# Zanue/EndoDAV

Measured on AMD Instinct MI355X. Metric: depth frames/sec (518x518, T=8 clip), higher is better.
Workload: dtype f32

## Files before the change

endodav_amd/csrc/temporal.hip:

```cpp
#include <cstdlib>

#include "ops.hpp"

namespace edv {
namespace {

using f32x4 = __attribute__((ext_vector_type(4))) float;

template <int TMAX>
__global__ __launch_bounds__(256) void attn_temporal_kernel(const float *__restrict__ qkv, float *__restrict__ out, int B, int T, int P, int C,
                                                             int heads, float scale) {
    const long long total = (long long)B * T * P * heads;
    const long long gid = (long long)blockIdx.x * 256 + threadIdx.x;
    if (gid >= total) return;
    const int head = (int)(gid % heads);
    long long r = gid / heads;
    const int p = (int)(r % P);
    r /= P;
    const int tq = (int)(r % T);
    const int b = (int)(r / T);
    const int d = C / heads, C3 = 3 * C;
    const long long tstride = (long long)P * C3;
    const float *qp = qkv + ((long long)(b * T + tq) * P + p) * C3 + head * d;
    const float *kb = qkv + ((long long)(b * T) * P + p) * C3 + C + head * d;
    const float *vb = kb + C;

    float s[TMAX];
#pragma unroll
    for (int ts = 0; ts < TMAX; ++ts) s[ts] = 0.f;
    for (int c = 0; c < d; c += 4) {
        const f32x4 q4 = *reinterpret_cast<const f32x4 *>(qp + c);
#pragma unroll
        for (int ts = 0; ts < TMAX; ++ts) {
            if (ts < T) {
                const f32x4 k4 = *reinterpret_cast<const f32x4 *>(kb + ts * tstride + c);
                s[ts] += (q4.x * k4.x + q4.y * k4.y) + (q4.z * k4.z + q4.w * k4.w);
            }
        }
    }
    float mx = -INFINITY;
#pragma unroll
    for (int ts = 0; ts < TMAX; ++ts)
        if (ts < T) {
            s[ts] *= scale;
            mx = fmaxf(mx, s[ts]);
        }
    float sum = 0.f;
#pragma unroll
    for (int ts = 0; ts < TMAX; ++ts)
        if (ts < T) {
            s[ts] = expf(s[ts] - mx);
            sum += s[ts];
        }
    const float inv = 1.0f / sum;
    float *op = out + ((long long)(b * T + tq) * P + p) * C + head * d;
    for (int c = 0; c < d; c += 4) {
        f32x4 acc = {0.f, 0.f, 0.f, 0.f};
#pragma unroll
        for (int ts = 0; ts < TMAX; ++ts)
            if (ts < T) acc += s[ts] * *reinterpret_cast<const f32x4 *>(vb + ts * tstride + c);
        *reinterpret_cast<f32x4 *>(op + c) = acc * inv;
    }
}

template <int TT>
__global__ __launch_bounds__(256) void attn_temporal_small_kernel(const float *__restrict__ qkv, float *__restrict__ out, int B, int T, int P, int C, int heads,
                                                                   float scale) {
    const long long total = (long long)B * P * heads;
    const long long gid = (long long)blockIdx.x * 256 + threadIdx.x;
    if (gid >= total) return;
    const int head = (int)(gid % heads);
    long long r = gid / heads;
    const int p = (int)(r % P);
    const int b = (int)(r / P);
    const int d = C / heads, C3 = 3 * C;
    const long long ts3 = (long long)P * C3, ts1 = (long long)P * C;
    const float *qb = qkv + ((long long)(b * T) * P + p) * C3 + head * d;
    const float *kb = qb + C, *vb = qb + 2 * C;
    float *ob = out + ((long long)(b * T) * P + p) * C + head * d;
    float S[TT][TT];
#pragma unroll
    for (int i = 0; i < TT; ++i)
#pragma unroll
        for (int j = 0; j < TT; ++j) S[i][j] = 0.f;
#pragma unroll 2
    for (int c = 0; c < d; c += 4) {
        f32x4 q4[TT], k4[TT];
#pragma unroll
        for (int t = 0; t < TT; ++t) {
            const int tc = t < T ? t : T - 1;
            q4[t] = *reinterpret_cast<const f32x4 *>(qb + tc * ts3 + c);
            k4[t] = *reinterpret_cast<const f32x4 *>(kb + tc * ts3 + c);
        }
#pragma unroll
        for (int i = 0; i < TT; ++i)
#pragma unroll
            for (int j = 0; j < TT; ++j) S[i][j] += (q4[i].x * k4[j].x + q4[i].y * k4[j].y) + (q4[i].z * k4[j].z + q4[i].w * k4[j].w);
    }
#pragma unroll
    for (int i = 0; i < TT; ++i) {
        float mx = -INFINITY;
#pragma unroll
        for (int j = 0; j < TT; ++j)
            if (j < T) {
                S[i][j] *= scale;
                mx = fmaxf(mx, S[i][j]);
            }
        float sum = 0.f;
#pragma unroll
        for (int j = 0; j < TT; ++j) {
            S[i][j] = j < T ? expf(S[i][j] - mx) : 0.f;
            sum += S[i][j];
        }
        const float inv = 1.0f / sum;
#pragma unroll
        for (int j = 0; j < TT; ++j) S[i][j] *= inv;
    }
#pragma unroll 2
    for (int c = 0; c < d; c += 4) {
        f32x4 v4[TT];
#pragma unroll
        for (int t = 0; t < TT; ++t) v4[t] = *reinterpret_cast<const f32x4 *>(vb + (t < T ? t : T - 1) * ts3 + c);
#pragma unroll
        for (int i = 0; i < TT; ++i) {
            if (i < T) {
                f32x4 acc = {0.f, 0.f, 0.f, 0.f};
#pragma unroll
                for (int j = 0; j < TT; ++j) acc += S[i][j] * v4[j];
                *reinterpret_cast<f32x4 *>(ob + i * ts1 + c) = acc;
            }
        }
    }
}

template <int TMAX>
__global__ __launch_bounds__(256) void attn_temporal_pixel_kernel(const float *__restrict__ qkv, float *__restrict__ out, int T, int P, int C, int heads,
                                                                   int HG, float scale) {
    extern __shared__ __attribute__((aligned(16))) float sm[];
    const int tid = threadIdx.x, nthr = blockDim.x;
    const int ngroups = heads / HG;
    const int hg = blockIdx.x % ngroups;
    const long long bp = blockIdx.x / ngroups;
    const int b = (int)(bp / P), p = (int)(bp - (long long)b * P);
    const int d = C / heads, C3 = 3 * C, W = HG * d, w4 = W >> 2;
    for (int idx = tid; idx < T * 3 * w4; idx += nthr) {
        const int t = idx / (3 * w4), r = idx - t * 3 * w4;
        const int part = r / w4, c4 = r - part * w4;
        *reinterpret_cast<f32x4 *>(&sm[(t * 3 + part) * W + 4 * c4]) =
            *reinterpret_cast<const f32x4 *>(qkv + ((long long)(b * T + t) * P + p) * C3 + part * C + hg * W + 4 * c4);
    }
    __syncthreads();
    const int hl = tid % HG, tq = tid / HG;
    if (tq >= T) return;
    const float *q = sm + (tq * 3 + 0) * W + hl * d;
    float s[TMAX];
#pragma unroll
    for (int ts = 0; ts < TMAX; ++ts) s[ts] = 0.f;
    for (int c = 0; c < d; c += 4) {
        const f32x4 q4 = *reinterpret_cast<const f32x4 *>(q + c);
#pragma unroll
        for (int ts = 0; ts < TMAX; ++ts)
            if (ts < T) {
                const f32x4 k4 = *reinterpret_cast<const f32x4 *>(sm + (ts * 3 + 1) * W + hl * d + c);
                s[ts] += (q4.x * k4.x + q4.y * k4.y) + (q4.z * k4.z + q4.w * k4.w);
            }
    }
    float mx = -INFINITY;
#pragma unroll
    for (int ts = 0; ts < TMAX; ++ts)
        if (ts < T) {
            s[ts] *= scale;
            mx = fmaxf(mx, s[ts]);
        }
    float sum = 0.f;
#pragma unroll
    for (int ts = 0; ts < TMAX; ++ts) {
        s[ts] = ts < T ? expf(s[ts] - mx) : 0.f;
        sum += s[ts];
    }
    const float inv = 1.0f / sum;
    float *op = out + ((long long)(b * T + tq) * P + p) * C + (hg * HG + hl) * d;
    for (int c = 0; c < d; c += 4) {
        f32x4 acc = {0.f, 0.f, 0.f, 0.f};
#pragma unroll
        for (int ts = 0; ts < TMAX; ++ts)
            if (ts < T) acc += s[ts] * *reinterpret_cast<const f32x4 *>(sm + (ts * 3 + 2) * W + hl * d + c);
        *reinterpret_cast<f32x4 *>(op + c) = acc * inv;
    }
}

__global__ __launch_bounds__(256) void geglu_kernel(const float *__restrict__ x, float *__restrict__ y, long long total4, int inner4) {
    for (long long i = (long long)blockIdx.x * 256 + threadIdx.x; i < total4; i += (long long)gridDim.x * 256) {
        const long long m = i / inner4;
        const int j = (int)(i - m * inner4);
        const float *row = x + m * (long long)inner4 * 8;
        const f32x4 a = *reinterpret_cast<const f32x4 *>(row + 4 * j);
        const f32x4 g = *reinterpret_cast<const f32x4 *>(row + 4 * (inner4 + j));
        f32x4 o = {a.x * gelu_erf(g.x), a.y * gelu_erf(g.y), a.z * gelu_erf(g.z), a.w * gelu_erf(g.w)};
        *reinterpret_cast<f32x4 *>(y + i * 4) = o;
    }
}


__global__ __launch_bounds__(256) void rope_qk_kernel(float *__restrict__ qkv, const float *__restrict__ table, long long n_pairs, int T, int P, int C,
                                                      float sign) {
    const long long i = (long long)blockIdx.x * 256 + threadIdx.x;
    if (i >= n_pairs) return;
    const int half = C >> 1;
    const long long m = i / half;
    const int j = (int)(i - m * half);
    const int t = (int)((m / P) % T);
    const float2 cs = *reinterpret_cast<const float2 *>(table + ((size_t)t * half + j) * 2);
    const float c = cs.x, sn = sign * cs.y;
    float2 *q = reinterpret_cast<float2 *>(qkv + m * 3 * C + 2 * j), *k = reinterpret_cast<float2 *>(qkv + m * 3 * C + C + 2 * j);
    const float2 a = *q, b = *k;
    *q = make_float2(a.x * c - a.y * sn, a.x * sn + a.y * c);
    *k = make_float2(b.x * c - b.y * sn, b.x * sn + b.y * c);
}

}

int attn_temporal(const float *qkv, float *out, int B, int T, int P, int C, int heads, hipStream_t st) {
    EDV_CHECK(qkv && out, "null operand");
    EDV_CHECK(B > 0 && T > 0 && P > 0 && C > 0 && heads > 0, "empty problem");
    EDV_CHECK(T <= 64, "T > 64 frames per clip is not built (temporal attention keeps a query's T scores in registers)");
    EDV_CHECK(C % heads == 0 && (C / heads) % 4 == 0, "head dim must be a multiple of 4");
    const long long total = (long long)B * T * P * heads;
    const long long blocks = (total + 255) / 256;
    EDV_CHECK(blocks < (1ll << 31), "grid");
    const float scale = 1.0f / sqrtf((float)(C / heads));
    dim3 grid((unsigned)blocks), block(256);
    static const bool per_query = [] {
        const char *e = getenv("EDV_TATTN_PER_QUERY");
        return e && atoi(e) != 0;
    }();
    const int d = C / heads;
    int HG = heads;
    while (HG > 1 && ((long long)T * HG > 256 || (size_t)T * 3 * HG * d * sizeof(float) > 64 * 1024 || heads % HG != 0)) --HG;
    const size_t lds_cap = (T > 32 && HG == 1) ? 160 * 1024 : 64 * 1024;
    const bool pixel_fits = (long long)T * HG <= 256 && (size_t)T * 3 * HG * d * sizeof(float) <= lds_cap && (long long)B * P * (heads / HG) < (1ll << 31);
    if (!per_query && pixel_fits && (T > 8 || d >= 24)) {
        const dim3 g3((unsigned)((long long)B * P * (heads / HG)));
        const dim3 b3((unsigned)(((T * HG + 63) / 64) * 64));
        const size_t lds = (size_t)T * 3 * HG * d * sizeof(float);
        if (T <= 8)
            EDV_LAUNCH(attn_temporal_pixel_kernel<8>, g3, b3, lds, st, qkv, out, T, P, C, heads, HG, scale);
        else if (T <= 16)
            EDV_LAUNCH(attn_temporal_pixel_kernel<16>, g3, b3, lds, st, qkv, out, T, P, C, heads, HG, scale);
        else if (T <= 32)
            EDV_LAUNCH(attn_temporal_pixel_kernel<32>, g3, b3, lds, st, qkv, out, T, P, C, heads, HG, scale);
        else {
            if (lds > 64 * 1024)
                EDV_HIP(hipFuncSetAttribute(reinterpret_cast<const void *>(attn_temporal_pixel_kernel<64>), hipFuncAttributeMaxDynamicSharedMemorySize, (int)lds_cap));
            EDV_LAUNCH(attn_temporal_pixel_kernel<64>, g3, b3, lds, st, qkv, out, T, P, C, heads, HG, scale);
        }
    } else if (T > 32) {
        EDV_CHECK(false, "temporal attention over more than 32 frames: one head's q|k|v of a pixel (T x 3 x C/8 floats) must fit the 160 KB of LDS");
    } else if (T <= 8 && !per_query) {
        const long long tot = (long long)B * P * heads;
        const dim3 g2((unsigned)((tot + 255) / 256));
        if (T <= 4)
            EDV_LAUNCH(attn_temporal_small_kernel<4>, g2, block, 0, st, qkv, out, B, T, P, C, heads, scale);
        else
            EDV_LAUNCH(attn_temporal_small_kernel<8>, g2, block, 0, st, qkv, out, B, T, P, C, heads, scale);
    } else if (T <= 8)
        EDV_LAUNCH(attn_temporal_kernel<8>, grid, block, 0, st, qkv, out, B, T, P, C, heads, scale);
    else if (T <= 16)
        EDV_LAUNCH(attn_temporal_kernel<16>, grid, block, 0, st, qkv, out, B, T, P, C, heads, scale);
    else
        EDV_LAUNCH(attn_temporal_kernel<32>, grid, block, 0, st, qkv, out, B, T, P, C, heads, scale);
    EDV_LAUNCH_OK();
    return 0;
}

int geglu(const float *x, float *y, long long M, int inner, hipStream_t st) {
    EDV_CHECK(x && y, "null operand");
    EDV_CHECK(M > 0 && inner > 0 && inner % 4 == 0, "shape");
    const long long total4 = M * (inner / 4);
    const int blocks = (int)((total4 + 255) / 256 < 8192 ? (total4 + 255) / 256 : 8192);
    EDV_LAUNCH(geglu_kernel, dim3(blocks), dim3(256), 0, st, x, y, total4, inner / 4);
    EDV_LAUNCH_OK();
    return 0;
}

int rope_qk(float *qkv, const float *table, int B, int T, int P, int C, bool transpose, hipStream_t st) {
    EDV_CHECK(qkv && table, "null operand");
    EDV_CHECK(B > 0 && T > 0 && P > 0 && C > 0 && C % 2 == 0, "bad shape");
    const long long n = (long long)B * T * P * (C / 2);
    EDV_LAUNCH(rope_qk_kernel, dim3((unsigned)((n + 255) / 256)), dim3(256), 0, st, qkv, table, n, T, P, C, transpose ? -1.f : 1.f);
    EDV_LAUNCH_OK();
    return 0;
}

}
```

Measured before the change: 1027.

## Add pixel-tiled temporal attention kernel staging multiple pixels per block in LDS

Adds a new temporal attention kernel that loads a tile of up to eight pixels times a group of heads for all T frames into shared memory. Loads are issued into registers before any LDS write, giving wider, more coalesced global reads. Each query's head dimension is split across several lanes, and the partial dot products are combined with xor shuffles. It is enabled by default through an env knob and replaces the previous one-pixel-per-block kernel, at the cost of more register pressure and extra index math.

New measurement: 1032, median of 6. Within noise of the previous version (+0.5%).

```diff
diff --git a/endodav_amd/csrc/temporal.hip b/endodav_amd/csrc/temporal.hip
--- a/endodav_amd/csrc/temporal.hip
+++ b/endodav_amd/csrc/temporal.hip
@@ -189,6 +189,93 @@
     }
 }
 
+__device__ __forceinline__ int div_small(int a, float inv) { return (int)(((float)a + 0.5f) * inv); }
+
+template <int TMAX, int NL>
+__global__ __launch_bounds__(256, TMAX == 32 ? 3 : 1) void attn_temporal_tile_kernel(const float *__restrict__ qkv, float *__restrict__ out, int T, int P, int C,
+                                                                                      int heads, int lpt, int lhg, int lsp, int tiles, int rs4, float inv_rw4,
+                                                                                      float inv_w4, float scale) {
+    extern __shared__ __attribute__((aligned(16))) f32x4 sm4[];
+    const int tid = threadIdx.x;
+    const int PT = 1 << lpt, HG = 1 << lhg, DS = 1 << lsp;
+    const int ngroups = heads >> lhg;
+    const int hg = blockIdx.x % ngroups;
+    const int bt = blockIdx.x / ngroups;
+    const int b = bt / tiles, p0 = (bt - b * tiles) << lpt;
+    const int d4 = (C / heads) >> 2, c4n = C >> 2, w4 = d4 << lhg, rw4 = 3 * w4;
+    const int n4 = (T << lpt) * rw4;
+    const f32x4 *src = reinterpret_cast<const f32x4 *>(qkv) + (long long)b * T * P * (3 * c4n) + hg * w4;
+    f32x4 v[NL];
+    int dst[NL];
+#pragma unroll
+    for (int i = 0; i < NL; ++i) {
+        const int slot = tid + i * 256;
+        const int idx = slot < n4 ? slot : n4 - 1;
+        const int row = div_small(idx, inv_rw4), r = idx - row * rw4;
+        const int part = div_small(r, inv_w4), c4 = r - part * w4;
+        const int t = row >> lpt, pp = p0 + (row & (PT - 1));
+        const int pc = pp < P ? pp : P - 1;
+        dst[i] = (slot < n4 && pp < P) ? row * rs4 + part * w4 + c4 : -1;
+        v[i] = src[((long long)t * P + pc) * (3 * c4n) + part * c4n + c4];
+    }
+#pragma unroll
+    for (int i = 0; i < NL; ++i)
+        if (dst[i] >= 0) sm4[dst[i]] = v[i];
+    __syncthreads();
+    const int nwork = T << (lpt + lhg + lsp), fs4 = rs4 << lpt;
+    for (int it = tid; it < nwork; it += 256) {
+        const int ds = it & (DS - 1), hl = (it >> lsp) & (HG - 1), pix = (it >> (lsp + lhg)) & (PT - 1), tq = it >> (lsp + lhg + lpt);
+        const int pp = p0 + pix;
+        if (pp >= P) continue;
+        const f32x4 *base = sm4 + pix * rs4 + hl * d4;
+        const f32x4 *q = base + tq * fs4;
+        float s[TMAX];
+#pragma unroll
+        for (int ts = 0; ts < TMAX; ++ts) s[ts] = 0.f;
+        for (int c = ds; c < d4; c += DS) {
+            const f32x4 q4 = q[c];
+#pragma unroll
+            for (int t0 = 0; t0 < TMAX; t0 += 8)
+                if (t0 < T) {
+#pragma unroll
+                    for (int ts = t0; ts < t0 + 8; ++ts) {
+                        const f32x4 k4 = base[(ts < T ? ts : T - 1) * fs4 + w4 + c];
+                        s[ts] += (q4.x * k4.x + q4.y * k4.y) + (q4.z * k4.z + q4.w * k4.w);
+                    }
+                }
+        }
+        for (int m = 1; m < DS; m <<= 1) {
+#pragma unroll
+            for (int ts = 0; ts < TMAX; ++ts) s[ts] += __shfl_xor(s[ts], m);
+        }
+        float mx = -INFINITY;
+#pragma unroll
+        for (int ts = 0; ts < TMAX; ++ts)
+            if (ts < T) {
+                s[ts] *= scale;
+                mx = fmaxf(mx, s[ts]);
+            }
+        float sum = 0.f;
+#pragma unroll
+        for (int ts = 0; ts < TMAX; ++ts) {
+            s[ts] = ts < T ? expf(s[ts] - mx) : 0.f;
+            sum += s[ts];
+        }
+        const float inv = 1.0f / sum;
+        f32x4 *op = reinterpret_cast<f32x4 *>(out) + ((long long)(b * T + tq) * P + pp) * c4n + ((hg << lhg) + hl) * d4;
+        for (int c = ds; c < d4; c += DS) {
+            f32x4 acc = {0.f, 0.f, 0.f, 0.f};
+#pragma unroll
+            for (int t0 = 0; t0 < TMAX; t0 += 8)
+                if (t0 < T) {
+#pragma unroll
+                    for (int ts = t0; ts < t0 + 8; ++ts) acc += s[ts] * base[(ts < T ? ts : T - 1) * fs4 + 2 * w4 + c];
+                }
+            op[c] = acc * inv;
+        }
+    }
+}
+
 __global__ __launch_bounds__(256) void geglu_kernel(const float *__restrict__ x, float *__restrict__ y, long long total4, int inner4) {
     for (long long i = (long long)blockIdx.x * 256 + threadIdx.x; i < total4; i += (long long)gridDim.x * 256) {
         const long long m = i / inner4;
@@ -218,6 +305,58 @@
     *k = make_float2(b.x * c - b.y * sn, b.x * sn + b.y * c);
 }
 
+constexpr size_t TILE_LDS = 48 * 1024;
+struct TilePlan {
+    int lpt, lhg, lsp, rs4, tiles, nl;
+    size_t bytes;
+    long long grid;
+};
+
+bool tile_plan(int B, int T, int P, int C, int heads, int pt_cap, TilePlan &pl) {
+    const int d = C / heads;
+    int lhg = 0;
+    while (lhg < 3 && heads % (2 << lhg) == 0) ++lhg;
+    while (lhg > 0 && (size_t)T * 3 * (d << lhg) * sizeof(float) > TILE_LDS) --lhg;
+    const int W = d << lhg;
+    if ((size_t)T * 3 * W * sizeof(float) > TILE_LDS) return false;
+    int lpt = 3;
+    while (lpt > 0 && ((1 << lpt) > pt_cap || (size_t)(T << lpt) * (3 * W + 4) * sizeof(float) > TILE_LDS)) --lpt;
+    pl.lpt = lpt;
+    pl.lhg = lhg;
+    pl.rs4 = 3 * (W >> 2) + (lpt > 0 ? 1 : 0);
+    pl.bytes = (size_t)(T << lpt) * pl.rs4 * 16;
+    const int n4 = (T << lpt) * 3 * (W >> 2);
+    pl.nl = ((n4 + 255) / 256 + 2) / 3 * 3;
+    int lsp = 0;
+    while (((T << (lpt + lhg + lsp)) << 1) <= 256 && (d >> 2) % (2 << lsp) == 0) ++lsp;
+    pl.lsp = lsp;
+    pl.tiles = (P + (1 << lpt) - 1) >> lpt;
+    pl.grid = (long long)B * pl.tiles * (heads >> lhg);
+    return pl.grid < (1ll << 31);
+}
+
+template <int TMAX>
+int launch_tile(const TilePlan &pl, const float *qkv, float *out, int T, int P, int C, int heads, float scale, hipStream_t st) {
+    const dim3 g((unsigned)pl.grid), b(256);
+    const int W = (C / heads) << pl.lhg;
+    const float inv_rw4 = 1.0f / (float)(3 * (W >> 2)), inv_w4 = 1.0f / (float)(W >> 2);
+#define EDV_TILE_CASE(NL)                                                                                                                  \
+    case NL:                                                                                                                               \
+        EDV_LAUNCH((attn_temporal_tile_kernel<TMAX, NL>), g, b, pl.bytes, st, qkv, out, T, P, C, heads, pl.lpt, pl.lhg, pl.lsp, pl.tiles, pl.rs4, inv_rw4, \
+                   inv_w4, scale);                                                                                                         \
+        break;
+    switch (pl.nl) {
+        EDV_TILE_CASE(3)
+        EDV_TILE_CASE(6)
+        EDV_TILE_CASE(9)
+        EDV_TILE_CASE(12)
+        default:
+            EDV_CHECK(false, "pixel-tile plan outside the instantiated loads per thread");
+    }
+#undef EDV_TILE_CASE
+    return 0;
+}
+
 }
 
 int attn_temporal(const float *qkv, float *out, int B, int T, int P, int C, int heads, hipStream_t st) {
@@ -234,6 +373,29 @@
         const char *e = getenv("EDV_TATTN_PER_QUERY");
         return e && atoi(e) != 0;
     }();
+    static const bool tile = [] {
+        const char *e = getenv("EDV_TATTN_TILE");
+        return !e || atoi(e) != 0;
+    }();
+    static const int tile_pt = [] {
+        const char *e = getenv("EDV_TATTN_TILE_PT");
+        return e && atoi(e) > 0 ? atoi(e) : 8;
+    }();
+    TilePlan pl;
+    if (!per_query && tile && tile_plan(B, T, P, C, heads, tile_pt, pl)) {
+        int rc;
+        if (T <= 8)
+            rc = launch_tile<8>(pl, qkv, out, T, P, C, heads, scale, st);
+        else if (T <= 16)
+            rc = launch_tile<16>(pl, qkv, out, T, P, C, heads, scale, st);
+        else if (T <= 32)
+            rc = launch_tile<32>(pl, qkv, out, T, P, C, heads, scale, st);
+        else
+            rc = launch_tile<64>(pl, qkv, out, T, P, C, heads, scale, st);
+        if (rc) return rc;
+        EDV_LAUNCH_OK();
+        return 0;
+    }
     const int d = C / heads;
     int HG = heads;
     while (HG > 1 && ((long long)T * HG > 256 || (size_t)T * 3 * HG * d * sizeof(float) > 64 * 1024 || heads % HG != 0)) --HG;
```
